# eloimoliner/BABE

Measured on AMD Instinct MI355X. Metric: audio-sec/s (blind BWE, 10 s @ 44.1 kHz clips, 35 EDM steps 2nd order), whole job, higher is better.
Workload: dtype f32

## Files before the change

### babe_amd/_lib.py

```python
import ctypes as C
import os

import torch

_HERE = os.path.dirname(os.path.abspath(__file__))
_LIB_PATH = os.environ.get("BABE_HIP_LIB") or os.path.join(_HERE, "libbabe_hip.so")
_lib = None


class BabeHipError(RuntimeError):
    pass


class ConvArgs(C.Structure):
    _fields_ = [
        ("in_", C.c_void_p), ("in_bs", C.c_long), ("in_cs", C.c_long),
        ("in2", C.c_void_p), ("in2_bs", C.c_long), ("in2_cs", C.c_long), ("cin_split", C.c_int),
        ("w_packed", C.c_void_p),
        ("out", C.c_void_p), ("out_bs", C.c_long), ("out_cs", C.c_long),
        ("res", C.c_void_p), ("res_bs", C.c_long), ("res_cs", C.c_long),
        ("in_scale", C.c_void_p), ("oscale", C.c_void_p),
        ("alpha", C.c_float), ("rbeta", C.c_float),
        ("B", C.c_int), ("Cin", C.c_int), ("Cout", C.c_int), ("F", C.c_int), ("T", C.c_int),
        ("KH", C.c_int), ("KW", C.c_int), ("dil", C.c_int),
# ... 48 lines not shown
    "babe_scale_gelu": [_P, _P, _P, _I, _I, _L, _P],
    "babe_units_size": [_I, _I, _I],
    "babe_scale_gelu_units": [_P, _P, _P, _I, _I, _I, _I, _P],
    "babe_conv2d_bf16_units_supported": [C.POINTER(ConvArgs)],
    "babe_conv2d_bf16_units": [C.POINTER(ConvArgs), _P, _P],
    "babe_gn_bwd_partial": [_P, _P, _P, _P, _I, _I, _I, _L, _I, _P],
    "babe_gn_bwd_apply": [_P, _P, _P, _P, _P, _P, _P, _F, _I, _I, _I, _L, _I, _F, _P],
    "babe_gn_bwd_apply_merge": [_P, _P, _P, _P, _P, _P, _P, _F, _I, _I, _I, _L, _I, _F, _P, _P, _F, _F],
    "babe_gn_bwd_partial_nogelu": [_P, _P, _P, _P, _I, _I, _I, _L, _I, _P],
    "babe_gn_bwd_apply_nogelu": [_P, _P, _P, _P, _P, _P, _P, _F, _I, _I, _I, _L, _I, _F, _P],
    "babe_attn_buckets": [_P, _I, _I, _I],
    "babe_attn_fwd": [_P, _P, _P, _P, _P, _I, _P, _P, _I, _I, _I, _I, _F, _P],
    "babe_attn_vjp": [_P, _P, _P, _P, _P, _I, _P, _P, _P, _P, _P, _P, _I, _I, _I, _I, _F, _P],
    "babe_resample": [_P, _L, _L, _P, _L, _L, _I, _I, _I, _I, _I, _F, _F, _P],
    "babe_resample_res": [_P, _L, _L, _P, _L, _L, _P, _L, _L, _I, _I, _I, _I, _I, _F, _F, _P],
    "babe_resample_sinc_adjoint": [_P, _L, _P, _L, _I, _L, _L, _P, _P, _I, _I, _I, _P],
    "babe_iir_filter": [_P, _L, _P, _L, _I, _L, _P, _P, _I, _I, _I, _P, _L, _P, _L, _P],
    "babe_decimate": [_P, _L, _P, _L, _I, _L, _L, _I, _I, _P],
    "babe_axpby4d": [_P, _L, _L, _P, _L, _L, _I, _I, _I, _I, _F, _F, _P],
    "babe_axpby2_4d": [_P, _L, _L, _P, _L, _L, _P, _L, _L, _I, _I, _I, _I, _F, _F, _P],
    "babe_linear": [_P, _P, _P, _P, _I, _I, _I, _I, _P],
    "babe_rff": [_P, _P, _P, _I, _I, _P],
    "babe_conv_wgrad_rows": [C.POINTER(WgradArgs), _P, _P, _F, _P, _P, _L, _F, _P, _L, _P],
    "babe_rows_sum": [_P, _L, _I, _L, _P, _F, _P],
    "babe_gn_param_grad": [_P, _P, _P, _P, _P, _P, _L, _F, _P, _L, _P, _L, _I, _I, _I, _L, _P],
    "babe_linear_bwd": [_P, _P, _P, _P, _P, _P, _P, _P, _I, _I, _I, _F, _P],
}


def lib():
    global _lib
    if _lib is None:
        if not os.path.exists(_LIB_PATH):
            raise BabeHipError(
# ... 107 lines not shown
```

### babe_amd/csrc/misc.hip

```cpp
#include "common.h"
#include "../../include/babe_hip.h"
#include "prof.h"
#include <cstdarg>
#include <vector>

static thread_local char g_err[512] = "";

void babe_set_error(const char* fmt, ...) {
    va_list ap;
    va_start(ap, fmt);
    vsnprintf(g_err, sizeof(g_err), fmt, ap);
    va_end(ap);
}
extern "C" const char* babe_last_error(void) { return g_err; }
extern "C" const char* babe_version(void) { return "babe_hip 0.1 (gfx950)"; }

namespace {
struct ProfRec { hipEvent_t e0, e1; int slot; void* stream; double flops; };
struct Prof {
    bool on = false;
    int conv_slot_override = -1;
    std::vector<ProfRec> rec;
    size_t used = 0;
    double bytes[BABE_NSLOTS] = {}, flops[BABE_NSLOTS] = {}, exec[BABE_NSLOTS] = {};
// ... 107 lines not shown
                                                      float* __restrict__ out, long out_bs, long out_cs, int C, long n,
                                                      float alpha, float beta) {
    const int b = blockIdx.y / C, c = blockIdx.y % C;
    const float* x = in + (long)b * in_bs + (long)c * in_cs;
    float* y = out + (long)b * out_bs + (long)c * out_cs;
    const long stride = (long)gridDim.x * blockDim.x * V;
    for (long i = ((long)blockIdx.x * blockDim.x + threadIdx.x) * V; i < n; i += stride) {
        if constexpr (V == 4) {
            typedef float f32x4 __attribute__((ext_vector_type(4)));
            f32x4 v = alpha * *reinterpret_cast<const f32x4*>(x + i);
            if (beta != 0.f) v += beta * *reinterpret_cast<const f32x4*>(y + i);
            *reinterpret_cast<f32x4*>(y + i) = v;
        } else {
            const float v = alpha * x[i];
            y[i] = (beta != 0.f) ? v + beta * y[i] : v;
        }
    }
}

__global__ __launch_bounds__(256) void axpby2_4d_kernel(const float* __restrict__ xin, long x_bs, long x_cs,
                                                        const float* __restrict__ yin, long y_bs, long y_cs,
                                                        float* __restrict__ out, long out_bs, long out_cs, int C, long n,
                                                        float alpha, float beta) {
    typedef float f32x4 __attribute__((ext_vector_type(4)));
    const int b = blockIdx.y / C, c = blockIdx.y % C;
    const float* x = xin + (long)b * x_bs + (long)c * x_cs;
    const float* y = yin + (long)b * y_bs + (long)c * y_cs;
    float* o = out + (long)b * out_bs + (long)c * out_cs;
    const long stride = (long)gridDim.x * blockDim.x * 4;
    for (long i = ((long)blockIdx.x * blockDim.x + threadIdx.x) * 4; i < n; i += stride) {
// ... 56 lines not shown
    if (v4) {
        int bx = cdiv(n / 4, 256);
        if (bx > 64) bx = 64;
        hipLaunchKernelGGL(axpby4d_kernel<4>, dim3(bx, B * C), dim3(256), 0, (hipStream_t)stream, in, in_bs, in_cs, out,
                           out_bs, out_cs, C, n, alpha, beta);
    } else {
        int bx = cdiv(n, 256);
        if (bx > 64) bx = 64;
        hipLaunchKernelGGL(axpby4d_kernel<1>, dim3(bx, B * C), dim3(256), 0, (hipStream_t)stream, in, in_bs, in_cs, out,
                           out_bs, out_cs, C, n, alpha, beta);
    }
    BABE_LAUNCH_CHECK();
    return BABE_OK;
}

extern "C" int babe_axpby2_4d(const float* x, long x_bs, long x_cs, const float* y, long y_bs, long y_cs, float* out, long out_bs,
                              long out_cs, int B, int C, int F, int T, float alpha, float beta, void* stream) {
    BABE_CHECK_ARG(x && y && out && B > 0 && C > 0 && F > 0 && T > 0, "axpby2_4d: bad arguments");
    BABE_CHECK_ARG((long)B * C <= 65535, "axpby2_4d: grid too large");
    const long n = (long)F * T;
    auto al16 = [](const void* p) { return ((uintptr_t)p & 15) == 0; };
    BABE_CHECK_ARG(n % 4 == 0 && al16(x) && al16(y) && al16(out) && x_bs % 4 == 0 && x_cs % 4 == 0 && y_bs % 4 == 0 && y_cs % 4 == 0 &&
                       out_bs % 4 == 0 && out_cs % 4 == 0,
                   "axpby2_4d: planes must be 16-byte aligned with F*T %% 4 == 0 (use two babe_axpby4d calls otherwise)");
    BabeProfScope prof(BABE_SLOT_AXPBY, 12.0 * B * C * (double)n, 0, 0, stream);
    int bx = cdiv(n / 4, 256);
    if (bx > 64) bx = 64;
    hipLaunchKernelGGL(axpby2_4d_kernel, dim3(bx, B * C), dim3(256), 0, (hipStream_t)stream, x, x_bs, x_cs, y, y_bs, y_cs, out, out_bs,
                       out_cs, C, n, alpha, beta);
    BABE_LAUNCH_CHECK();
// ... 31 lines not shown
```

### babe_amd/csrc/resample.hip

```cpp
#include "common.h"
#include "../../include/babe_hip.h"
#include "prof.h"

namespace {
__constant__ float kH[8] = {-0.01171875f, -0.03515625f, 0.11328125f, 0.43359375f,
                            0.43359375f,  0.11328125f,  -0.03515625f, -0.01171875f};

__device__ __forceinline__ int refl(int j, int T) { return j < 0 ? -j : (j >= T ? 2 * (T - 1) - j : j); }

__device__ __forceinline__ float down_gpad(const float* gy, int i, int Th) {
    float s = 0.f;
#pragma unroll
    for (int k = 0; k < 8; ++k) {
        const int d = i - k;
        if (d >= 0 && !(d & 1) && (d >> 1) < Th) s += kH[k] * gy[d >> 1];
    }
    return s;
}
__device__ __forceinline__ float up_gpad(const float* gy, int j, int T2) {
    float s = 0.f;
#pragma unroll
    for (int k = 0; k < 8; ++k) {
        const int n = 2 * j + k - 7;
        if (n >= 0 && n < T2) s += kH[k] * gy[n];
// ... 21 lines not shown
        if (n >= 1 && n <= 3) s += down_gpad(x, 3 - n, Th);
        if (n >= T - 4 && n <= T - 2) s += down_gpad(x, 2 * T + 1 - n, Th);
    } else {
        const int T2 = 2 * T;
        s = up_gpad(x, n + 2, T2);
        if (n >= 1 && n <= 2) s += up_gpad(x, 2 - n, T2);
        if (n >= T - 3 && n <= T - 2) s += up_gpad(x, 2 * T - n, T2);
    }
    return s;
}

template <int V, int VI>
__global__ __launch_bounds__(256) void resample_kernel(const float* __restrict__ in, long in_bs, long in_cs,
                                                       float* __restrict__ out, long out_bs, long out_cs, int C, int F,
                                                       int T, int mode, float alpha, float beta, int tout_shift,
                                                       const float* res, long res_bs, long res_cs) {
    const int b = blockIdx.y / C, c = blockIdx.y % C;
    const int Tin = (mode == 0 || mode == 1) ? T : (mode == 2 ? T / 2 : 2 * T);
    const int Tout = (mode == 0) ? T / 2 : (mode == 1 ? 2 * T : T);
    const unsigned i = (blockIdx.x * blockDim.x + threadIdx.x) * (unsigned)V;
    if (i >= (unsigned)(F * Tout)) return;
    const int f = tout_shift >= 0 ? (int)(i >> tout_shift) : (int)(i / (unsigned)Tout);
    const int n0 = (int)(i - (unsigned)f * (unsigned)Tout);
    const float* x = in + (long)b * in_bs + (long)c * in_cs + (long)f * Tin;
    float* y = out + (long)b * out_bs + (long)c * out_cs + (long)f * Tout + n0;
    const float* ry = res ? res + (long)b * res_bs + (long)c * res_cs + (long)f * Tout + n0 : y;
    float s[V];
    if constexpr (V == 4) {
        if (mode == 0 || mode == 3) {
            float w[14];
            const int base = 2 * n0 - 3;
            const bool inner = base >= 0 && base + 13 <= Tin - 1;
            if (inner) {
                if (VI && base - 1 >= 0 && base + 14 <= Tin - 1) {
                    typedef float f32x4 __attribute__((ext_vector_type(4)));
                    const f32x4* p4 = reinterpret_cast<const f32x4*>(x + base - 1);
                    const f32x4 q0 = p4[0], q1 = p4[1], q2 = p4[2], q3 = p4[3];
                    const float X[16] = {q0[0], q0[1], q0[2], q0[3], q1[0], q1[1], q1[2], q1[3],
                                         q2[0], q2[1], q2[2], q2[3], q3[0], q3[1], q3[2], q3[3]};
// ... 102 lines not shown
#pragma unroll
        for (int v = 0; v < V; ++v) s[v] = alpha * resample_one(x, n0 + v, T, mode);
    }
    if constexpr (V == 4) {
        typedef float f32x4 __attribute__((ext_vector_type(4)));
        f32x4 o = {s[0], s[1], s[2], s[3]};
        if (beta != 0.f) o += beta * *reinterpret_cast<const f32x4*>(ry);
        *reinterpret_cast<f32x4*>(y) = o;
    } else {
        y[0] = (beta != 0.f) ? s[0] + beta * ry[0] : s[0];
    }
}
}

static int resample_launch(const float* in, long in_bs, long in_cs, float* out, long out_bs, long out_cs, const float* res,
                           long res_bs, long res_cs, int B, int C, int F, int T, int mode, float alpha, float beta, void* stream) {
    BABE_CHECK_ARG(in && out && B > 0 && C > 0 && F > 0, "resample: bad arguments");
    BABE_CHECK_ARG(!res || ((((uintptr_t)res & 15) == 0) && res_bs % 4 == 0 && res_cs % 4 == 0 && (((uintptr_t)out & 15) == 0) &&
                            out_bs % 4 == 0 && out_cs % 4 == 0),
                   "resample_res: res / out must be 16-byte aligned views");
    BABE_CHECK_ARG(mode >= 0 && mode <= 3, "resample: bad mode %d", mode);
    BABE_CHECK_ARG(T >= 8 && (T % 2) == 0, "resample: T=%d unsupported (need even T >= 8)", T);
    BABE_CHECK_ARG((long)B * C <= 65535, "resample: grid too large");
    const int Tout = (mode == 0) ? T / 2 : (mode == 1 ? 2 * T : T);
    const bool v4 = (Tout % 4 == 0) && (((uintptr_t)out & 15) == 0) && (out_bs % 4 == 0) && (out_cs % 4 == 0);
    const long total = (long)F * Tout;
    BABE_CHECK_ARG(total < (1L << 31), "resample: plane too large");
    int tsh = -1;
    for (int k = 0; k < 31; ++k)
        if ((1 << k) == Tout) tsh = k;
    BabeProfScope prof(BABE_SLOT_RESAMPLE, 4.0 * B * C * (double)F * ((mode == 0 || mode == 1 ? T : (mode == 2 ? T / 2 : 2 * T)) + (beta != 0.f ? 2 : 1) * (double)Tout), 0, 0, stream);
    const int Tin = (mode == 0 || mode == 1) ? T : (mode == 2 ? T / 2 : 2 * T);
    const bool vin = (Tin % 4 == 0) && (((uintptr_t)in & 15) == 0) && (in_bs % 4 == 0) && (in_cs % 4 == 0);
    if (v4 && vin)
        hipLaunchKernelGGL((resample_kernel<4, 1>), dim3(cdiv(total / 4, 256), B * C), dim3(256), 0, (hipStream_t)stream, in,
                           in_bs, in_cs, out, out_bs, out_cs, C, F, T, mode, alpha, beta, tsh, res, res_bs, res_cs);
    else if (v4)
        hipLaunchKernelGGL((resample_kernel<4, 0>), dim3(cdiv(total / 4, 256), B * C), dim3(256), 0, (hipStream_t)stream, in,
                           in_bs, in_cs, out, out_bs, out_cs, C, F, T, mode, alpha, beta, tsh, res, res_bs, res_cs);
    else
        hipLaunchKernelGGL((resample_kernel<1, 0>), dim3(cdiv(total, 256), B * C), dim3(256), 0, (hipStream_t)stream, in,
                           in_bs, in_cs, out, out_bs, out_cs, C, F, T, mode, alpha, beta, tsh, res, res_bs, res_cs);
    BABE_LAUNCH_CHECK();
    return BABE_OK;
}

extern "C" int babe_resample(const float* in, long in_bs, long in_cs, float* out, long out_bs, long out_cs, int B,
                             int C, int F, int T, int mode, float alpha, float beta, void* stream) {
    return resample_launch(in, in_bs, in_cs, out, out_bs, out_cs, nullptr, 0, 0, B, C, F, T, mode, alpha, beta, stream);
}

extern "C" int babe_resample_res(const float* in, long in_bs, long in_cs, const float* res, long res_bs, long res_cs, float* out,
                                 long out_bs, long out_cs, int B, int C, int F, int T, int mode, float alpha, float beta,
                                 void* stream) {
    BABE_CHECK_ARG(res, "resample_res: null res");
    return resample_launch(in, in_bs, in_cs, out, out_bs, out_cs, res, res_bs, res_cs, B, C, F, T, mode, alpha, beta, stream);
}
```

### babe_amd/csrc/unet_engine.hip

```cpp
#include "common.h"
#include "../../include/babe_hip.h"
#include <cmath>
#include <cstdlib>
#include <cstring>

extern "C" int babe_conv2d_auto(babe_conv_args* a, const babe_packed_conv* pc, int transpose, void* stream) {
    BABE_CHECK_ARG(a && pc, "conv2d_auto: null arguments");
    a->Cin = transpose ? pc->Cout : pc->Cin;
    a->Cout = transpose ? pc->Cin : pc->Cout;
    a->KH = pc->KH;
    a->KW = pc->KW;
    const void* wq = transpose ? pc->bwd : pc->fwd;
    BABE_CHECK_ARG(wq, "conv2d_auto: weights not packed for this direction");
    if (!a->in2) a->cin_split = a->Cin;
    if (pc->splits) {
        a->w_packed = nullptr;
        a->stat_mode = 0;
        return babe_conv2d_bf16(a, wq, pc->splits, stream);
    }
    a->w_packed = (const float*)wq;
    const float* w45 = transpose ? pc->bwd_wino45 : pc->fwd_wino45;
    if (pc->w_raw && a->Cout <= 4 && babe_conv2d_fewco_supported(a)) {
        a->stat_mode = 0;
        return babe_conv2d_fewco(a, pc->w_raw, transpose, stream);
// ... 93 lines not shown
        a.B = B(); a.F = x.F; a.T = x.T; a.dil = dil;
        if (stat_part) { a.stat_mode = 1; a.stat_cg = stat_cg; a.stat_part = stat_part; }
        ck(babe_conv2d_auto(&a, &pc, transpose ? 1 : 0, st));
        return a.stat_mode == 1;
    }
    static int stat_slots(int cg, int F, int T, int dil) {
        babe_conv_args a;
        memset(&a, 0, sizeof a);
        a.stat_cg = cg; a.F = F; a.T = T; a.dil = dil;
        return babe_conv2d_wino85_stat_slots(&a);
    }
    void axpby(const View& x, const View& out, float alpha = 1.f, float beta = 0.f) {
        if (dry() || err) return;
        ck(babe_axpby4d(x.p, x.bs, x.cs, out.p, out.bs, out.cs, B(), x.C, x.F, x.T, alpha, beta, st));
    }
    static bool al16(const View& v) { return ((uintptr_t)v.p & 15) == 0 && v.bs % 4 == 0 && v.cs % 4 == 0; }
    void axpby2(const View& x, const View& y, const View& out, float alpha, float beta) {
        if (dry() || err) return;
        if (((long)x.F * x.T) % 4 == 0 && al16(x) && al16(y) && al16(out))
            ck(babe_axpby2_4d(x.p, x.bs, x.cs, y.p, y.bs, y.cs, out.p, out.bs, out.cs, B(), x.C, x.F, x.T, alpha, beta, st));
        else {
            axpby(x, out, alpha);
            axpby(y, out, beta, 1.f);
        }
    }
    void resample(const View& x, const View& out, int mode, float alpha = 1.f, float beta = 0.f, const View* res = nullptr) {
        if (dry() || err) return;
        const int T = mode == 0 || mode == 1 ? x.T : (mode == 2 ? x.T * 2 : x.T / 2);
        if (res) {
            if (al16(*res) && al16(out)) {
                ck(babe_resample_res(x.p, x.bs, x.cs, res->p, res->bs, res->cs, out.p, out.bs, out.cs, B(), x.C, x.F, T, mode, alpha, beta, st));
                return;
            }
            axpby(*res, out);
        }
        ck(babe_resample(x.p, x.bs, x.cs, out.p, out.bs, out.cs, B(), x.C, x.F, T, mode, alpha, beta, st));
    }
    static int splits(long n) { long s = n / 16384; return (int)(s < 1 ? 1 : (s > 64 ? 64 : s)); }
    const float* film_at(int off) const { return S->film + off; }

    View block_fwd(const babe_unet_block& blk, Saved* saved, const View& x, const View& out, const View* x2) {
        const int N = blk.N, Fq = x.F, T = x.T;
        View z;
        if (blk.proj_in.Cout) {
            z = buf(N, Fq, T);
            conv(x, blk.proj_in, z, 1, false, x2, nullptr, nullptr, nullptr, 1.f, 0.f);
        } else if (x.dense()) {
            z = x;
        } else {
            z = buf(N, Fq, T);
            axpby(x, z);
// ... 58 lines not shown
        a.B = B(); a.F = src.F; a.T = src.T; a.dil = dil;
        if (fuse_gn() && blk.k53 && cg % 4 == 0 && z.dense() && da.dense()) {
            a.stat_mode = 2; a.stat_cg = cg; a.stat_x = z.p; a.stat_scale = sv.scale; a.stat_part = *part;
        }
        ck(babe_conv2d_auto(&a, &blk.H[d], 1, st));
        return a.stat_mode == 2 ? Sf : 0;
    }
    static bool fuse_gn_fwd() {
        static const bool on = [] { const char* e = getenv("BABE_FUSE_GN_FWD"); return !(e && atoi(e) == 0); }();
        return on;
    }
    static bool fuse_gn() {
        static const bool on = [] { const char* e = getenv("BABE_FUSE_GN"); return e && atoi(e) != 0; }();
        return on;
    }
    void gn_bwd(const Saved& sv, const View& da, const View& gy, const View& gx, float rbeta, const View* acc, double* part, int Sf) {
        const View& z = sv.z;
        const long n = (long)(z.C / G_GROUPS) * z.F * z.T;
        const int Sp = Sf > 0 ? Sf : splits(n);
        if (dry() || err) return;
        if (Sf <= 0) ck(babe_gn_bwd_partial(z.p, da.p, sv.scale, part, B(), z.C, G_GROUPS, (long)z.F * z.T, Sp, st));
        if (acc)
            ck(babe_gn_bwd_apply_merge(z.p, da.p, gy.p, sv.scale, sv.stats, part, gx.p, rbeta, B(), z.C, G_GROUPS, (long)z.F * z.T, Sp, GN_EPS, st,
                                       acc->p, RS2, RS2));
        else
            ck(babe_gn_bwd_apply(z.p, da.p, gy.p, sv.scale, sv.stats, part, gx.p, rbeta, B(), z.C, G_GROUPS, (long)z.F * z.T, Sp, GN_EPS, st));
    }
    View block_vjp(const babe_unet_block& blk, const Saved* saved, const View& g_out, const View& g_in, bool accumulate, bool consume) {
        const int N = blk.N, Fq = g_out.F, T = g_out.T;
        const float beta = accumulate ? 1.f : 0.f;
        auto da_view = [&]() { View v; v.p = scratch_a((size_t)B() * N * Fq * T); v.C = N; v.F = Fq; v.T = T; v.cs = (long)Fq * T; v.bs = (long)N * Fq * T; return v; };
        if (!blk.res_conv.Cout && !blk.proj_out.Cout && !blk.proj_in.Cout && !accumulate && blk.nd > 0 && g_out.dense()) {
            View gz;
            if (blk.nd > 1) gz = buf(N, Fq, T);
            View da = da_view();
            View src = g_out;
            const bool merged = g_in.dense() && al16(g_in) && al16(g_out);
            for (int d = blk.nd - 1; d >= 0; --d) {
                double* part;
// ... 12 lines not shown
        if (blk.res_conv.Cout) conv(g_out, blk.res_conv, g_in, 1, true, nullptr, accumulate ? &g_in : nullptr, nullptr, nullptr, RS2, beta);
        else axpby(g_out, g_in, RS2, beta);
        float c = 1.f;
        View gz;
        if (blk.proj_out.Cout) {
            gz = buf(N, Fq, T);
            conv(g_out, blk.proj_out, gz, 1, true, nullptr, nullptr, nullptr, nullptr, RS2, 0.f);
        } else if (consume && g_out.dense()) {
            gz = g_out;
            c = RS2;
        } else {
            gz = buf(N, Fq, T);
            axpby(g_out, gz, RS2);
        }
        View da = da_view();
        for (int d = blk.nd - 1; d >= 0; --d) {
            double* part;
            const int Sf = conv_vjp(gz, blk, d, da, saved[d], &part);
            gn_bwd(saved[d], da, gz, gz, RS2, nullptr, part, Sf);
        }
        if (blk.proj_in.Cout) conv(gz, blk.proj_in, g_in, 1, true, nullptr, &g_in, nullptr, nullptr, c, 1.f);
        else axpby(gz, g_in, c, 1.f);
        return g_in;
    }

    void forward(const float* const* C_in, float** outs) {
        const int n = P->nocts, bpo = P->bpo;
        const int* Ns = P->Ns;
        const int* Ts = S->Ts;
        auto cview = [&](int lvl) { View v; v.p = const_cast<float*>(C_in[n - 1 - lvl]); v.C = 2; v.F = bpo; v.T = Ts[lvl]; v.cs = (long)bpo * Ts[lvl]; v.bs = 2 * v.cs; return v; };
        View XC = buf(Ns[0], bpo, Ts[0]);
        View pyr_prev, X;
        for (int i = 0; i < n; ++i) {
            const View C = cview(i);
            const int Fi = bpo * (i + 1);
            block_fwd(P->init_blk[i], S->saved[0][i], C, sub_f(XC, 0, bpo), nullptr);
            View pyr;
// ... 27 lines not shown
        {
            View Xm = buf(X.C, X.F, X.T);
            block_fwd(P->mid_blk, S->saved[4][0], X, Xm, nullptr);
            X = Xm;
        }
        View Xout = buf(2, bpo * n, Ts[n - 1]);
        block_fwd(P->mid_out, S->saved[5][0], X, Xout, nullptr);
        for (int i = 0; i < n; ++i) {
            const int j = n - 1 - i;
            const int Fj = bpo * (j + 1);
            const int Nout = Ns[j > 0 ? j - 1 : 0];
            View R = buf(Nout, Fj, Ts[j]);
            block_fwd(P->up_blk[i], S->saved[3][i], X, R, &S->hs[j]);
            View O = buf(2, Fj, Ts[j]);
            block_fwd(P->up_out[i], S->saved[2][i], R, O, nullptr);
            axpby(O, Xout, RS2, RS2);
            View o; o.p = outs[i]; o.C = 2; o.F = bpo; o.T = Ts[j]; o.cs = (long)bpo * Ts[j]; o.bs = 2 * o.cs;
            axpby(sub_f(Xout, 0, bpo), o);
            if (j > 0) {
                View Xn = buf(Nout, Fj - bpo, Ts[j - 1]);
                resample(sub_f(R, bpo, Fj - bpo), Xn, 1);
                View Xo = buf(2, Fj - bpo, Ts[j - 1]);
                resample(sub_f(Xout, bpo, Fj - bpo), Xo, 1);
                X = Xn;
                Xout = Xo;
            }
        }
    }

    void vjp(const float* const* gouts, float** gC) {
        const int n = P->nocts, bpo = P->bpo;
        const int* Ns = P->Ns;
        const int* Ts = S->Ts;
        View gH[8];
        View gX_prev, gXO_prev;
        for (int j = 0; j < n; ++j) {
            const int i = n - 1 - j;
            const int Fj = bpo * (j + 1);
            const int Nout = Ns[j > 0 ? j - 1 : 0];
            View gXOn = buf(2, Fj, Ts[j]);
            View gcat = buf(2 * Ns[j], Fj, Ts[j]);
            const size_t lvl = mark();
            View gXOp = buf(2, Fj, Ts[j]);
            View go; go.p = const_cast<float*>(gouts[i]); go.C = 2; go.F = bpo; go.T = Ts[j]; go.cs = (long)bpo * Ts[j]; go.bs = 2 * go.cs;
            axpby(go, sub_f(gXOp, 0, bpo));
            View gR = buf(Nout, Fj, Ts[j]);
            bool accumulate = false;
            if (j > 0) {
                resample(gXO_prev, sub_f(gXOp, bpo, Fj - bpo), 3);
                if (!dry() && !err) ck(babe_fill4d(gR.p, gR.bs, gR.cs, B(), Nout, bpo, Ts[j], 0.f, st));
                resample(gX_prev, sub_f(gR, bpo, Fj - bpo), 3);
                accumulate = true;
            }
            View gO = buf(2, Fj, Ts[j]);
            axpby(gXOp, gO, RS2);
            block_vjp(P->up_out[i], S->saved[2][i], gO, gR, accumulate, true);
            axpby(gXOp, gXOn, RS2);
            gXO_prev = gXOn;
            block_vjp(P->up_blk[i], S->saved[3][i], gR, gcat, false, true);
            gX_prev = sub_c(gcat, 0, Ns[j]);
            gH[j] = sub_c(gcat, Ns[j], Ns[j]);
            release(lvl);
        }
        View gM = buf(Ns[n - 1], bpo * n, Ts[n - 1]);
        axpby(gX_prev, gM);
        block_vjp(P->mid_out, S->saved[5][0], gXO_prev, gM, true, true);
        View gXm = buf(gM.C, gM.F, gM.T);
        block_vjp(P->mid_blk, S->saved[4][0], gM, gXm, false, true);
        View gpyr_next, gP;
        bool have_next = false;
        for (int i = n - 1; i >= 0; --i) {
            const int Fi = bpo * (i + 1);
// ... 128 lines not shown
```

### babe_amd/networks/unet_engine.py

```python
import math
import os

import torch

from .. import ops

RS2 = 1.0 / math.sqrt(2.0)
USE_C = os.environ.get("BABE_UNET_C", "0") == "1"
MERGE_TAIL = os.environ.get("BABE_MERGE_TAIL", "1") != "0"


class _Attn:

    def __init__(self, g, Fdim, N, film_index, opts):
        self.H, self.bias_qkv, self.rel_pos, self.nbk, self.maxd = opts
        self.F = Fdim
        self.scale = float(Fdim) ** -0.5
        self.gamma = g("norm2.gamma").reshape(-1).contiguous()
        self.film_off = (film_index.add(g("affine2.weight"), g("affine2.bias")), film_index.add(g("gate2.weight"), g("gate2.bias")))
        self.proj_in = ops.PackedConv(g("attn_block.proj_in.weight"))
        self.proj_out = ops.PackedConv(g("attn_block.proj_out.weight"))
        w = g("attn_block.qk.weight")
        self.qk = ops.PackedConv(w.reshape(w.shape[0], w.shape[1], 1, 1))
        self.qk_bias = g("attn_block.qk.bias").contiguous() if self.bias_qkv else None
# ... 356 lines not shown
            blk.saved = None
            blk.inp = blk.zpo = None
            return g_in
        if blk.res_conv is not None:
            ops.conv2d(g_out, blk.res_conv, g_in, transpose=True, alpha=RS2, rbeta=beta, res=g_in if accumulate else None)
        else:
            ops.axpby(g_out, g_in, alpha=RS2, beta=beta)
        c = 1.0
        if blk.proj_out is not None:
            gz = ops.conv2d(g_out, blk.proj_out, self.buf(B, N, Fq, T), transpose=True, alpha=RS2)
        elif consume and g_out.is_contiguous():
            gz, c = g_out, RS2
        else:
            gz = ops.axpby(g_out, self.buf(B, N, Fq, T), alpha=RS2)
        da = self.scratch("a", B * N * Fq * T).view(B, N, Fq, T)
        for d in reversed(range(blk.nd)):
            z, stats, scale, gate = blk.saved[d]
            if pg is not None:
                self._layer_wgrad(pg, blk, d, gz, c)
            fs = ops.conv2d(gz, blk.H[d], da, dil=blk.dil(d), transpose=True, in_scale=gate, alpha=RS2, vjp_stat=(z, scale, N // 8))
            if pg is not None:
                self._layer_gn_grad(pg, blk, d, da, c)
            ops.gn_bwd(z, da, gz, scale, stats, gz, RS2, fused=fs)
        if blk.attn is not None:
            self.attn_vjp(blk, gz, c)
            c = 1.0
        if pg is not None and blk.proj_in is not None:
            x, x2 = blk.inp
            self._wg(pg, blk.p + "proj_in.weight", x, gz, blk.proj_in, c, x2=x2)
        if blk.proj_in is not None:
            ops.conv2d(gz, blk.proj_in, g_in, transpose=True, res=g_in, alpha=c, rbeta=1.0)
        else:
            ops.axpby(gz, g_in, alpha=c, beta=1.0)
        blk.saved = None
        blk.inp = blk.zpo = None
        return g_in

    def _c_engine(self):
        if not USE_C or self.precision != "f32" or self.has_attention:
            return None
        cu = self.__dict__.get("_cunet")
        if cu is None:
            from .unet_c import CUnet
            parent = self.__dict__.get("_cunet_parent")
            cu = parent.clone(self) if parent is not None else CUnet(self)
            self._cunet = cu
        return cu
# ... 39 lines not shown
                ops.resample(H, sub, 0)
                ops.conv2d(pyr, self.pyr_conv[i], sub, res=sub, alpha=RS2, rbeta=RS2)
                XC = XCn
            else:
                X = ops.conv2d(pyr, self.pyr_conv[i], self.buf(B, Ns[i], Fi, Ts[i]), res=H, alpha=RS2, rbeta=RS2)
        self.hs = hs
        X = self.block_fwd(self.mid_blk, X, film, self.buf(*X.shape))
        Xout = self.block_fwd(self.mid_out, X, film, self.buf(B, 2, bpo * n, Ts[-1]))
        outs = [None] * n
        for i in range(n):
            j = n - 1 - i
            Fj = bpo * (j + 1)
            Nout = Ns[max(j - 1, 0)]
            R = self.block_fwd(self.up_blk[i], X, film, self.buf(B, Nout, Fj, Ts[j]), x2=hs[j])
            O = self.block_fwd(self.up_out[i], R, film, self.buf(B, 2, Fj, Ts[j]))
            ops.axpby(O, Xout, alpha=RS2, beta=RS2)
            outs[i] = ops.axpby(Xout[:, :, :bpo, :], self.buf(B, 2, bpo, Ts[j]))
            if j > 0:
                X = ops.resample(R[:, :, bpo:, :], self.buf(B, Nout, Fj - bpo, Ts[j - 1]), 1)
                Xout = ops.resample(Xout[:, :, bpo:, :], self.buf(B, 2, Fj - bpo, Ts[j - 1]), 1)
        return outs

    def vjp(self, gouts, pg=None):
        assert pg is None or self._train, "parameter gradients need forward(..., train=True)"
        if getattr(self, "_c_fwd", False):
            return self._c_engine().vjp([g.contiguous() for g in gouts])
        n, bpo, Ns, Ts, B = self.nocts, self.bpo, self.Ns, self.Ts, self.B
        gH = [None] * n
        gX_prev = gXO_prev = None
        for j in range(n):
            i = n - 1 - j
            Fj = bpo * (j + 1)
            Nout = Ns[max(j - 1, 0)]
            gXOp = self.buf(B, 2, Fj, Ts[j])
            ops.axpby(gouts[i], gXOp[:, :, :bpo, :])
            gR = self.buf(B, Nout, Fj, Ts[j])
            if j > 0:
                ops.resample(gXO_prev, gXOp[:, :, bpo:, :], 3)
                gR[:, :, :bpo, :].zero_()
                ops.resample(gX_prev, gR[:, :, bpo:, :], 3)
                accumulate = True
            else:
                accumulate = False
            gO = ops.axpby(gXOp, self.buf(B, 2, Fj, Ts[j]), alpha=RS2)
            self.block_vjp(self.up_out[i], gO, gR, accumulate=accumulate, consume=True, pg=pg)
            gXO_prev = ops.axpby(gXOp, self.buf(B, 2, Fj, Ts[j]), alpha=RS2)
            gcat = self.buf(B, 2 * Ns[j], Fj, Ts[j])
            self.block_vjp(self.up_blk[i], gR, gcat, consume=True, pg=pg)
            gX_prev = gcat[:, :Ns[j]]
            gH[j] = gcat[:, Ns[j]:]
        gM = self.buf(B, Ns[-1], bpo * n, Ts[-1])
        ops.axpby(gX_prev, gM)
        self.block_vjp(self.mid_out, gXO_prev, gM, accumulate=True, consume=True, pg=pg)
        gXm = self.block_vjp(self.mid_blk, gM, self.buf(*gM.shape), consume=True, pg=pg)
        gC = [None] * n
        gpyr_next = None
        gP = None
        for i in reversed(range(n)):
            Fi = bpo * (i + 1)
            if pg is not None:
                self._wg(pg, f"downs.{i}.1.weight", self.pyrs[i], gXm if i == n - 1 else gP, self.pyr_conv[i], RS2)
# ... 28 lines not shown
```

### babe_amd/ops.py

```python
import ctypes as C
import math
import os

import torch

from . import _lib
from ._lib import ConvArgs, CPackedConv, WgradArgs, check, lib, ptr, stream

RSQRT2 = 1.0 / math.sqrt(2.0)


def _view(t):
    assert t.dim() == 4 and t.dtype == torch.float32
    assert t.stride(3) == 1 and t.stride(2) == t.shape[3], f"rows must be contiguous, got strides {t.stride()}"
    return ptr(t), t.stride(0), t.stride(1)


PRECISIONS = {"f32": 0, "bf16": 1, "bf16x3": 2}
BF16_HBM_F32 = os.environ.get("BABE_BF16_HBM_F32", "1") != "0"
_W = os.environ.get("BABE_CONV_WINO", "4")
FEWCO = os.environ.get("BABE_CONV_FEWCO", "1") != "0"
WINOGRAD = _W != "0"
WINOGRAD4 = _W not in ("0", "2", "1")
WINOGRAD45 = WINOGRAD4 and os.environ.get("BABE_CONV_WINO45", "1") != "0"
# ... 326 lines not shown
    assert out.shape == (B, Cc, F, Tout), (out.shape, (B, Cc, F, Tout))
    xp, xbs, xcs = _view(x)
    op, obs, ocs = _view(out)
    if res is not None:
        assert res.shape == out.shape
        rp, rbs, rcs = _view(res)
        if AXPBY2 and all(v % 4 == 0 for v in (rbs, rcs, obs, ocs)) and res.data_ptr() % 16 == 0 and out.data_ptr() % 16 == 0:
            check(lib().babe_resample_res(xp, xbs, xcs, rp, rbs, rcs, op, obs, ocs, B, Cc, F, T, mode, alpha, beta, stream()),
                  "resample_res")
            return out
        axpby(res, out)
    check(lib().babe_resample(xp, xbs, xcs, op, obs, ocs, B, Cc, F, T, mode, alpha, beta, stream()), "resample")
    return out


def axpby(x, out, alpha=1.0, beta=0.0):
    assert x.shape == out.shape
    B, Cc, F, T = x.shape
    xp, xbs, xcs = _view(x)
    op, obs, ocs = _view(out)
    check(lib().babe_axpby4d(xp, xbs, xcs, op, obs, ocs, B, Cc, F, T, alpha, beta, stream()), "axpby4d")
    return out


def axpby2(x, y, out, alpha, beta):
    assert x.shape == out.shape and y.shape == out.shape
    B, Cc, F, T = x.shape
    xp, xbs, xcs = _view(x)
    yp, ybs, ycs = _view(y)
    op, obs, ocs = _view(out)
# ... 146 lines not shown
```

### include/babe_hip.h

```cpp
#ifndef BABE_HIP_H
#define BABE_HIP_H
#ifdef __cplusplus
extern "C" {
#endif

const char* babe_version(void);
const char* babe_last_error(void);

typedef struct { float* p; long bs; long cs; } babe_view;

typedef struct {
    const float* in;  long in_bs,  in_cs;
    const float* in2; long in2_bs, in2_cs; int cin_split;
    const float* w_packed;
    float* out;       long out_bs, out_cs;
    const float* res; long res_bs, res_cs;
    const float* in_scale;
    const float* oscale;
    float alpha, rbeta;
    int B, Cin, Cout, F, T, KH, KW, dil;
    int stat_mode, stat_cg;
    const float* stat_x; const float* stat_scale; double* stat_part;
} babe_conv_args;
int babe_conv2d_wino85_stat_slots(const babe_conv_args* a);
// ... 55 lines not shown
                      int B, int C, int G, long hw, int S, float eps, void* stream);
int babe_gn_bwd_apply_merge(const float* x, const float* da, const float* gy, const float* scale,
                            const float* stats, const double* part, float* gx, float rbeta,
                            int B, int C, int G, long hw, int S, float eps, void* stream,
                            const float* acc, float ca, float cb);
int babe_gn_bwd_partial_nogelu(const float* x, const float* da, const float* scale, double* part, int B, int C, int G, long hw,
                               int S, void* stream);
int babe_gn_bwd_apply_nogelu(const float* x, const float* da, const float* gy, const float* scale, const float* stats,
                             const double* part, float* gx, float rbeta, int B, int C, int G, long hw, int S, float eps,
                             void* stream);

int babe_resample(const float* in, long in_bs, long in_cs, float* out, long out_bs, long out_cs,
                  int B, int C, int F, int T, int mode, float alpha, float beta, void* stream);
int babe_resample_res(const float* in, long in_bs, long in_cs, const float* res, long res_bs, long res_cs, float* out,
                      long out_bs, long out_cs, int B, int C, int F, int T, int mode, float alpha, float beta, void* stream);

int babe_resample_sinc(const float* x, long x_bs, float* out, long out_bs, int B, long L_in, long L_out, const float* kernel,
                       const int* krange, int orig, int new_, int width, void* stream);
int babe_resample_sinc_adjoint(const float* g, long g_bs, float* out, long out_bs, int B, long L_in, long L_out,
                               const float* kernel, const int* krange, int orig, int new_, int width, void* stream);

long babe_iir_workspace(int B, long L, int order);
int babe_iir_filter(const float* x, long x_bs, float* y, long y_bs, int B, long L, const float* b, const float* a, int order,
                    int clamp, int adjoint, unsigned char* mask, long mask_bs, void* workspace, long workspace_bytes, void* stream);
int babe_decimate(const float* in, long in_bs, float* out, long out_bs, int B, long L_full, long L_dec, int factor, int adjoint,
                  void* stream);

long babe_conv_packed_size_wino85(int Cout, int Cin, int transpose_flip);
int babe_conv_pack_weights_wino85(const float* w, float* dst, int Cout, int Cin, int KH, int KW, int transpose_flip, void* stream);
int babe_conv2d_wino85_supported(const babe_conv_args* a);
// ... 20 lines not shown
    int Ns[8];
    babe_unet_block init_blk[8], main_blk[8], up_out[8], up_blk[8], mid_blk, mid_out;
    babe_packed_conv pyr_conv[8];
} babe_unet_plan_desc;
void* babe_unet_plan_create(const babe_unet_plan_desc* desc);
void babe_unet_plan_destroy(void* plan);
void* babe_unet_state_create(void);
void babe_unet_state_destroy(void* state);
long babe_unet_workspace_bytes(const void* plan, int B, const int* T_oct);
int babe_unet_fwd(const void* plan, void* state, const float* const* C_in, const float* film, long film_bs, int B,
                  const int* T_oct, void* workspace, long workspace_bytes, float* const* outs, void* stream);
int babe_unet_vjp(const void* plan, void* state, const float* const* gouts, float* const* gC, void* stream);

int babe_axpby4d(const float* in, long in_bs, long in_cs, float* out, long out_bs, long out_cs,
                 int B, int C, int F, int T, float alpha, float beta, void* stream);
int babe_fill4d(float* out, long out_bs, long out_cs, int B, int C, int F, int T, float value, void* stream);
int babe_axpby2_4d(const float* x, long x_bs, long x_cs, const float* y, long y_bs, long y_cs, float* out, long out_bs,
                   long out_cs, int B, int C, int F, int T, float alpha, float beta, void* stream);

int babe_linear(const float* x, const float* W, const float* bias, float* out, int B, int K, int J,
                int relu, void* stream);
int babe_rff(const float* cnoise, const float* freq, float* out, int B, int R, void* stream);

int babe_rfft_mixed(const float* x_in, float* spec_out, const float* spec_in, float* x_out, float* work, int B, int N1,
                    int N2, int K2, const int* rad1, int nrad1, const int* rad2, int nrad2, const float* w1, const float* w2,
                    const float* tw, int direction, void* stream);
int babe_fft_twiddle_transpose(const float* in, float* out, const float* tw, int B, int N1, int N2,
                               int adjoint, void* stream);
typedef struct {
    int nbands; int L; int KX;
// ... 156 lines not shown
```

Baseline: 2.548.

## Fuse elementwise copies, zero-fill and tail axpby into neighbouring UNet kernels

Several small elementwise passes in the UNet forward and VJP are folded into adjacent kernels. The output-add and copy-out become a single dual-store axpby. The zero-fill of the leading rows joins the upsampling resample. The RS2 scale moves into the gradient copy and resample, which removes two temporary buffers. The final residual axpby in the block VJP is merged into the last group-norm backward apply. These changes cut kernel launches and memory traffic, at the cost of more special-case code paths and argument plumbing that must stay correct.

```diff
diff --git a/babe_amd/_lib.py b/babe_amd/_lib.py
--- a/babe_amd/_lib.py
+++ b/babe_amd/_lib.py
@@ -86,10 +86,12 @@
     "babe_attn_vjp": [_P, _P, _P, _P, _P, _I, _P, _P, _P, _P, _P, _P, _I, _I, _I, _I, _F, _P],
     "babe_resample": [_P, _L, _L, _P, _L, _L, _I, _I, _I, _I, _I, _F, _F, _P],
     "babe_resample_res": [_P, _L, _L, _P, _L, _L, _P, _L, _L, _I, _I, _I, _I, _I, _F, _F, _P],
+    "babe_resample_zrows": [_P, _L, _L, _P, _L, _L, _I, _I, _I, _I, _I, _F, _I, _P],
     "babe_resample_sinc_adjoint": [_P, _L, _P, _L, _I, _L, _L, _P, _P, _I, _I, _I, _P],
     "babe_iir_filter": [_P, _L, _P, _L, _I, _L, _P, _P, _I, _I, _I, _P, _L, _P, _L, _P],
     "babe_decimate": [_P, _L, _P, _L, _I, _L, _L, _I, _I, _P],
     "babe_axpby4d": [_P, _L, _L, _P, _L, _L, _I, _I, _I, _I, _F, _F, _P],
+    "babe_axpby4d_dup": [_P, _L, _L, _P, _L, _L, _P, _L, _L, _I, _I, _I, _I, _I, _F, _F, _P],
     "babe_axpby2_4d": [_P, _L, _L, _P, _L, _L, _P, _L, _L, _I, _I, _I, _I, _F, _F, _P],
     "babe_linear": [_P, _P, _P, _P, _I, _I, _I, _I, _P],
     "babe_rff": [_P, _P, _P, _I, _I, _P],
diff --git a/babe_amd/csrc/misc.hip b/babe_amd/csrc/misc.hip
--- a/babe_amd/csrc/misc.hip
+++ b/babe_amd/csrc/misc.hip
@@ -145,6 +145,32 @@
         } else {
             const float v = alpha * x[i];
             y[i] = (beta != 0.f) ? v + beta * y[i] : v;
+        }
+    }
+}
+
+template <int V>
+__global__ __launch_bounds__(256) void axpby4d_dup_kernel(const float* __restrict__ in, long in_bs, long in_cs,
+                                                          float* __restrict__ out, long out_bs, long out_cs,
+                                                          float* __restrict__ out2, long out2_bs, long out2_cs, int C, long n,
+                                                          long n2, float alpha, float beta) {
+    const int b = blockIdx.y / C, c = blockIdx.y % C;
+    const float* x = in + (long)b * in_bs + (long)c * in_cs;
+    float* y = out + (long)b * out_bs + (long)c * out_cs;
+    float* y2 = out2 + (long)b * out2_bs + (long)c * out2_cs;
+    const long stride = (long)gridDim.x * blockDim.x * V;
+    for (long i = ((long)blockIdx.x * blockDim.x + threadIdx.x) * V; i < n; i += stride) {
+        if constexpr (V == 4) {
+            typedef float f32x4 __attribute__((ext_vector_type(4)));
+            f32x4 v = alpha * *reinterpret_cast<const f32x4*>(x + i);
+            if (beta != 0.f) v += beta * *reinterpret_cast<const f32x4*>(y + i);
+            *reinterpret_cast<f32x4*>(y + i) = v;
+            if (i < n2) *reinterpret_cast<f32x4*>(y2 + i) = v;
+        } else {
+            float v = alpha * x[i];
+            if (beta != 0.f) v = v + beta * y[i];
+            y[i] = v;
+            if (i < n2) y2[i] = v;
         }
     }
 }
@@ -231,6 +257,30 @@
     return BABE_OK;
 }
 
+extern "C" int babe_axpby4d_dup(const float* in, long in_bs, long in_cs, float* out, long out_bs, long out_cs, float* out2,
+                                long out2_bs, long out2_cs, int B, int C, int F, int T, int F2, float alpha, float beta, void* stream) {
+    BABE_CHECK_ARG(in && out && out2 && B > 0 && C > 0 && F > 0 && T > 0 && F2 > 0 && F2 <= F, "axpby4d_dup: bad arguments");
+    BABE_CHECK_ARG((long)B * C <= 65535 && F <= 65535, "axpby4d_dup: grid too large");
+    const long n = (long)F * T, n2 = (long)F2 * T;
+    auto al16 = [](const void* p) { return ((uintptr_t)p & 15) == 0; };
+    const bool v4 = (n % 4 == 0) && (n2 % 4 == 0) && al16(in) && al16(out) && al16(out2) && in_bs % 4 == 0 && in_cs % 4 == 0 &&
+                    out_bs % 4 == 0 && out_cs % 4 == 0 && out2_bs % 4 == 0 && out2_cs % 4 == 0;
+    BabeProfScope prof(BABE_SLOT_AXPBY, ((beta != 0.f ? 12.0 : 8.0) * (double)n + 4.0 * (double)n2) * B * C, 0, 0, stream);
+    if (v4) {
+        int bx = cdiv(n / 4, 256);
+        if (bx > 64) bx = 64;
+        hipLaunchKernelGGL(axpby4d_dup_kernel<4>, dim3(bx, B * C), dim3(256), 0, (hipStream_t)stream, in, in_bs, in_cs, out,
+                           out_bs, out_cs, out2, out2_bs, out2_cs, C, n, n2, alpha, beta);
+    } else {
+        int bx = cdiv(n, 256);
+        if (bx > 64) bx = 64;
+        hipLaunchKernelGGL(axpby4d_dup_kernel<1>, dim3(bx, B * C), dim3(256), 0, (hipStream_t)stream, in, in_bs, in_cs, out,
+                           out_bs, out_cs, out2, out2_bs, out2_cs, C, n, n2, alpha, beta);
+    }
+    BABE_LAUNCH_CHECK();
+    return BABE_OK;
+}
+
 extern "C" int babe_axpby2_4d(const float* x, long x_bs, long x_cs, const float* y, long y_bs, long y_cs, float* out, long out_bs,
                               long out_cs, int B, int C, int F, int T, float alpha, float beta, void* stream) {
     BABE_CHECK_ARG(x && y && out && B > 0 && C > 0 && F > 0 && T > 0, "axpby2_4d: bad arguments");
diff --git a/babe_amd/csrc/resample.hip b/babe_amd/csrc/resample.hip
--- a/babe_amd/csrc/resample.hip
+++ b/babe_amd/csrc/resample.hip
@@ -59,15 +59,25 @@
 __global__ __launch_bounds__(256) void resample_kernel(const float* __restrict__ in, long in_bs, long in_cs,
                                                        float* __restrict__ out, long out_bs, long out_cs, int C, int F,
                                                        int T, int mode, float alpha, float beta, int tout_shift,
-                                                       const float* res, long res_bs, long res_cs) {
+                                                       const float* res, long res_bs, long res_cs, int zrows) {
     const int b = blockIdx.y / C, c = blockIdx.y % C;
     const int Tin = (mode == 0 || mode == 1) ? T : (mode == 2 ? T / 2 : 2 * T);
     const int Tout = (mode == 0) ? T / 2 : (mode == 1 ? 2 * T : T);
     const unsigned i = (blockIdx.x * blockDim.x + threadIdx.x) * (unsigned)V;
-    if (i >= (unsigned)(F * Tout)) return;
+    if (i >= (unsigned)((F + zrows) * Tout)) return;
     const int f = tout_shift >= 0 ? (int)(i >> tout_shift) : (int)(i / (unsigned)Tout);
     const int n0 = (int)(i - (unsigned)f * (unsigned)Tout);
-    const float* x = in + (long)b * in_bs + (long)c * in_cs + (long)f * Tin;
+    if (f < zrows) {
+        float* z = out + (long)b * out_bs + (long)c * out_cs + (long)f * Tout + n0;
+        if constexpr (V == 4) {
+            typedef float f32x4 __attribute__((ext_vector_type(4)));
+            *reinterpret_cast<f32x4*>(z) = f32x4{0.f, 0.f, 0.f, 0.f};
+        } else {
+            z[0] = 0.f;
+        }
+        return;
+    }
+    const float* x = in + (long)b * in_bs + (long)c * in_cs + (long)(f - zrows) * Tin;
     float* y = out + (long)b * out_bs + (long)c * out_cs + (long)f * Tout + n0;
     const float* ry = res ? res + (long)b * res_bs + (long)c * res_cs + (long)f * Tout + n0 : y;
     float s[V];
@@ -200,7 +210,8 @@
 }
 
 static int resample_launch(const float* in, long in_bs, long in_cs, float* out, long out_bs, long out_cs, const float* res,
-                           long res_bs, long res_cs, int B, int C, int F, int T, int mode, float alpha, float beta, void* stream) {
+                           long res_bs, long res_cs, int B, int C, int F, int T, int mode, float alpha, float beta, void* stream,
+                           int zrows = 0) {
     BABE_CHECK_ARG(in && out && B > 0 && C > 0 && F > 0, "resample: bad arguments");
     BABE_CHECK_ARG(!res || ((((uintptr_t)res & 15) == 0) && res_bs % 4 == 0 && res_cs % 4 == 0 && (((uintptr_t)out & 15) == 0) &&
                             out_bs % 4 == 0 && out_cs % 4 == 0),
@@ -210,7 +221,7 @@
     BABE_CHECK_ARG((long)B * C <= 65535, "resample: grid too large");
     const int Tout = (mode == 0) ? T / 2 : (mode == 1 ? 2 * T : T);
     const bool v4 = (Tout % 4 == 0) && (((uintptr_t)out & 15) == 0) && (out_bs % 4 == 0) && (out_cs % 4 == 0);
-    const long total = (long)F * Tout;
+    const long total = (long)(F + zrows) * Tout;
     BABE_CHECK_ARG(total < (1L << 31), "resample: plane too large");
     int tsh = -1;
     for (int k = 0; k < 31; ++k)
@@ -220,13 +231,13 @@
     const bool vin = (Tin % 4 == 0) && (((uintptr_t)in & 15) == 0) && (in_bs % 4 == 0) && (in_cs % 4 == 0);
     if (v4 && vin)
         hipLaunchKernelGGL((resample_kernel<4, 1>), dim3(cdiv(total / 4, 256), B * C), dim3(256), 0, (hipStream_t)stream, in,
-                           in_bs, in_cs, out, out_bs, out_cs, C, F, T, mode, alpha, beta, tsh, res, res_bs, res_cs);
+                           in_bs, in_cs, out, out_bs, out_cs, C, F, T, mode, alpha, beta, tsh, res, res_bs, res_cs, zrows);
     else if (v4)
         hipLaunchKernelGGL((resample_kernel<4, 0>), dim3(cdiv(total / 4, 256), B * C), dim3(256), 0, (hipStream_t)stream, in,
-                           in_bs, in_cs, out, out_bs, out_cs, C, F, T, mode, alpha, beta, tsh, res, res_bs, res_cs);
+                           in_bs, in_cs, out, out_bs, out_cs, C, F, T, mode, alpha, beta, tsh, res, res_bs, res_cs, zrows);
     else
         hipLaunchKernelGGL((resample_kernel<1, 0>), dim3(cdiv(total, 256), B * C), dim3(256), 0, (hipStream_t)stream, in,
-                           in_bs, in_cs, out, out_bs, out_cs, C, F, T, mode, alpha, beta, tsh, res, res_bs, res_cs);
+                           in_bs, in_cs, out, out_bs, out_cs, C, F, T, mode, alpha, beta, tsh, res, res_bs, res_cs, zrows);
     BABE_LAUNCH_CHECK();
     return BABE_OK;
 }
@@ -242,3 +253,9 @@
     BABE_CHECK_ARG(res, "resample_res: null res");
     return resample_launch(in, in_bs, in_cs, out, out_bs, out_cs, res, res_bs, res_cs, B, C, F, T, mode, alpha, beta, stream);
 }
+
+extern "C" int babe_resample_zrows(const float* in, long in_bs, long in_cs, float* out, long out_bs, long out_cs, int B, int C, int F,
+                                   int T, int mode, float alpha, int zrows, void* stream) {
+    BABE_CHECK_ARG(zrows >= 0, "resample_zrows: bad zrows");
+    return resample_launch(in, in_bs, in_cs, out, out_bs, out_cs, nullptr, 0, 0, B, C, F, T, mode, alpha, 0.f, stream, zrows);
+}
diff --git a/babe_amd/csrc/unet_engine.hip b/babe_amd/csrc/unet_engine.hip
--- a/babe_amd/csrc/unet_engine.hip
+++ b/babe_amd/csrc/unet_engine.hip
@@ -131,6 +131,10 @@
         if (dry() || err) return;
         ck(babe_axpby4d(x.p, x.bs, x.cs, out.p, out.bs, out.cs, B(), x.C, x.F, x.T, alpha, beta, st));
     }
+    void axpby_dup(const View& x, const View& out, const View& out2, float alpha, float beta) {
+        if (dry() || err) return;
+        ck(babe_axpby4d_dup(x.p, x.bs, x.cs, out.p, out.bs, out.cs, out2.p, out2.bs, out2.cs, B(), x.C, x.F, x.T, out2.F, alpha, beta, st));
+    }
     static bool al16(const View& v) { return ((uintptr_t)v.p & 15) == 0 && v.bs % 4 == 0 && v.cs % 4 == 0; }
     void axpby2(const View& x, const View& y, const View& out, float alpha, float beta) {
         if (dry() || err) return;
@@ -152,6 +156,11 @@
             axpby(*res, out);
         }
         ck(babe_resample(x.p, x.bs, x.cs, out.p, out.bs, out.cs, B(), x.C, x.F, T, mode, alpha, beta, st));
+    }
+    void resample_zrows(const View& x, const View& out, int mode, int zrows, float alpha = 1.f) {
+        if (dry() || err) return;
+        const int T = mode == 0 || mode == 1 ? x.T : (mode == 2 ? x.T * 2 : x.T / 2);
+        ck(babe_resample_zrows(x.p, x.bs, x.cs, out.p, out.bs, out.cs, B(), x.C, x.F, T, mode, alpha, zrows, st));
     }
     static int splits(long n) { long s = n / 16384; return (int)(s < 1 ? 1 : (s > 64 ? 64 : s)); }
     const float* film_at(int off) const { return S->film + off; }
@@ -240,7 +249,8 @@
         static const bool on = [] { const char* e = getenv("BABE_FUSE_GN"); return e && atoi(e) != 0; }();
         return on;
     }
-    void gn_bwd(const Saved& sv, const View& da, const View& gy, const View& gx, float rbeta, const View* acc, double* part, int Sf) {
+    void gn_bwd(const Saved& sv, const View& da, const View& gy, const View& gx, float rbeta, const View* acc, double* part, int Sf,
+                float ca = RS2, float cb = RS2) {
         const View& z = sv.z;
         const long n = (long)(z.C / G_GROUPS) * z.F * z.T;
         const int Sp = Sf > 0 ? Sf : splits(n);
@@ -248,7 +258,7 @@
         if (Sf <= 0) ck(babe_gn_bwd_partial(z.p, da.p, sv.scale, part, B(), z.C, G_GROUPS, (long)z.F * z.T, Sp, st));
         if (acc)
             ck(babe_gn_bwd_apply_merge(z.p, da.p, gy.p, sv.scale, sv.stats, part, gx.p, rbeta, B(), z.C, G_GROUPS, (long)z.F * z.T, Sp, GN_EPS, st,
-                                       acc->p, RS2, RS2));
+                                       acc->p, ca, cb));
         else
             ck(babe_gn_bwd_apply(z.p, da.p, gy.p, sv.scale, sv.stats, part, gx.p, rbeta, B(), z.C, G_GROUPS, (long)z.F * z.T, Sp, GN_EPS, st));
     }
@@ -291,13 +301,15 @@
             axpby(g_out, gz, RS2);
         }
         View da = da_view();
+        const bool tail_merged = !blk.proj_in.Cout && blk.nd > 0 && g_in.C == N && g_in.dense() && al16(g_in);
         for (int d = blk.nd - 1; d >= 0; --d) {
             double* part;
             const int Sf = conv_vjp(gz, blk, d, da, saved[d], &part);
-            gn_bwd(saved[d], da, gz, gz, RS2, nullptr, part, Sf);
+            if (d == 0 && tail_merged) gn_bwd(saved[d], da, gz, g_in, RS2, &g_in, part, Sf, 1.f, c);
+            else gn_bwd(saved[d], da, gz, gz, RS2, nullptr, part, Sf);
         }
         if (blk.proj_in.Cout) conv(gz, blk.proj_in, g_in, 1, true, nullptr, &g_in, nullptr, nullptr, c, 1.f);
-        else axpby(gz, g_in, c, 1.f);
+        else if (!tail_merged) axpby(gz, g_in, c, 1.f);
         return g_in;
     }
 
@@ -355,9 +367,8 @@
             block_fwd(P->up_blk[i], S->saved[3][i], X, R, &S->hs[j]);
             View O = buf(2, Fj, Ts[j]);
             block_fwd(P->up_out[i], S->saved[2][i], R, O, nullptr);
-            axpby(O, Xout, RS2, RS2);
             View o; o.p = outs[i]; o.C = 2; o.F = bpo; o.T = Ts[j]; o.cs = (long)bpo * Ts[j]; o.bs = 2 * o.cs;
-            axpby(sub_f(Xout, 0, bpo), o);
+            axpby_dup(O, Xout, o, RS2, RS2);
             if (j > 0) {
                 View Xn = buf(Nout, Fj - bpo, Ts[j - 1]);
                 resample(sub_f(R, bpo, Fj - bpo), Xn, 1);
@@ -382,21 +393,16 @@
             View gXOn = buf(2, Fj, Ts[j]);
             View gcat = buf(2 * Ns[j], Fj, Ts[j]);
             const size_t lvl = mark();
-            View gXOp = buf(2, Fj, Ts[j]);
             View go; go.p = const_cast<float*>(gouts[i]); go.C = 2; go.F = bpo; go.T = Ts[j]; go.cs = (long)bpo * Ts[j]; go.bs = 2 * go.cs;
-            axpby(go, sub_f(gXOp, 0, bpo));
+            axpby(go, sub_f(gXOn, 0, bpo), RS2);
             View gR = buf(Nout, Fj, Ts[j]);
             bool accumulate = false;
             if (j > 0) {
-                resample(gXO_prev, sub_f(gXOp, bpo, Fj - bpo), 3);
-                if (!dry() && !err) ck(babe_fill4d(gR.p, gR.bs, gR.cs, B(), Nout, bpo, Ts[j], 0.f, st));
-                resample(gX_prev, sub_f(gR, bpo, Fj - bpo), 3);
+                resample(gXO_prev, sub_f(gXOn, bpo, Fj - bpo), 3, RS2);
+                resample_zrows(gX_prev, gR, 3, bpo);
                 accumulate = true;
             }
-            View gO = buf(2, Fj, Ts[j]);
-            axpby(gXOp, gO, RS2);
-            block_vjp(P->up_out[i], S->saved[2][i], gO, gR, accumulate, true);
-            axpby(gXOp, gXOn, RS2);
+            block_vjp(P->up_out[i], S->saved[2][i], gXOn, gR, accumulate, false);
             gXO_prev = gXOn;
             block_vjp(P->up_blk[i], S->saved[3][i], gR, gcat, false, true);
             gX_prev = sub_c(gcat, 0, Ns[j]);
diff --git a/babe_amd/networks/unet_engine.py b/babe_amd/networks/unet_engine.py
--- a/babe_amd/networks/unet_engine.py
+++ b/babe_amd/networks/unet_engine.py
@@ -394,6 +394,8 @@
         else:
             gz = ops.axpby(g_out, self.buf(B, N, Fq, T), alpha=RS2)
         da = self.scratch("a", B * N * Fq * T).view(B, N, Fq, T)
+        tail_merged = (blk.proj_in is None and blk.attn is None and blk.nd > 0 and g_in.shape[1] == N and g_in.is_contiguous()
+                       and g_in.data_ptr() % 16 == 0)
         for d in reversed(range(blk.nd)):
             z, stats, scale, gate = blk.saved[d]
             if pg is not None:
@@ -401,7 +403,10 @@
             fs = ops.conv2d(gz, blk.H[d], da, dil=blk.dil(d), transpose=True, in_scale=gate, alpha=RS2, vjp_stat=(z, scale, N // 8))
             if pg is not None:
                 self._layer_gn_grad(pg, blk, d, da, c)
-            ops.gn_bwd(z, da, gz, scale, stats, gz, RS2, fused=fs)
+            if d == 0 and tail_merged:
+                ops.gn_bwd(z, da, gz, scale, stats, g_in, RS2, merge=(g_in, 1.0, c), fused=fs)
+            else:
+                ops.gn_bwd(z, da, gz, scale, stats, gz, RS2, fused=fs)
         if blk.attn is not None:
             self.attn_vjp(blk, gz, c)
             c = 1.0
@@ -410,7 +415,7 @@
             self._wg(pg, blk.p + "proj_in.weight", x, gz, blk.proj_in, c, x2=x2)
         if blk.proj_in is not None:
             ops.conv2d(gz, blk.proj_in, g_in, transpose=True, res=g_in, alpha=c, rbeta=1.0)
-        else:
+        elif not tail_merged:
             ops.axpby(gz, g_in, alpha=c, beta=1.0)
         blk.saved = None
         blk.inp = blk.zpo = None
@@ -480,8 +485,8 @@
             Nout = Ns[max(j - 1, 0)]
             R = self.block_fwd(self.up_blk[i], X, film, self.buf(B, Nout, Fj, Ts[j]), x2=hs[j])
             O = self.block_fwd(self.up_out[i], R, film, self.buf(B, 2, Fj, Ts[j]))
-            ops.axpby(O, Xout, alpha=RS2, beta=RS2)
-            outs[i] = ops.axpby(Xout[:, :, :bpo, :], self.buf(B, 2, bpo, Ts[j]))
+            outs[i] = self.buf(B, 2, bpo, Ts[j])
+            ops.axpby_dup(O, Xout, outs[i], alpha=RS2, beta=RS2)
             if j > 0:
                 X = ops.resample(R[:, :, bpo:, :], self.buf(B, Nout, Fj - bpo, Ts[j - 1]), 1)
                 Xout = ops.resample(Xout[:, :, bpo:, :], self.buf(B, 2, Fj - bpo, Ts[j - 1]), 1)
@@ -498,19 +503,17 @@
             i = n - 1 - j
             Fj = bpo * (j + 1)
             Nout = Ns[max(j - 1, 0)]
-            gXOp = self.buf(B, 2, Fj, Ts[j])
-            ops.axpby(gouts[i], gXOp[:, :, :bpo, :])
+            gXOn = self.buf(B, 2, Fj, Ts[j])
+            ops.axpby(gouts[i], gXOn[:, :, :bpo, :], alpha=RS2)
             gR = self.buf(B, Nout, Fj, Ts[j])
             if j > 0:
-                ops.resample(gXO_prev, gXOp[:, :, bpo:, :], 3)
-                gR[:, :, :bpo, :].zero_()
-                ops.resample(gX_prev, gR[:, :, bpo:, :], 3)
+                ops.resample(gXO_prev, gXOn[:, :, bpo:, :], 3, alpha=RS2)
+                ops.resample_zrows(gX_prev, gR, 3, bpo)
                 accumulate = True
             else:
                 accumulate = False
-            gO = ops.axpby(gXOp, self.buf(B, 2, Fj, Ts[j]), alpha=RS2)
-            self.block_vjp(self.up_out[i], gO, gR, accumulate=accumulate, consume=True, pg=pg)
-            gXO_prev = ops.axpby(gXOp, self.buf(B, 2, Fj, Ts[j]), alpha=RS2)
+            self.block_vjp(self.up_out[i], gXOn, gR, accumulate=accumulate, pg=pg)
+            gXO_prev = gXOn
             gcat = self.buf(B, 2 * Ns[j], Fj, Ts[j])
             self.block_vjp(self.up_blk[i], gR, gcat, consume=True, pg=pg)
             gX_prev = gcat[:, :Ns[j]]
diff --git a/babe_amd/ops.py b/babe_amd/ops.py
--- a/babe_amd/ops.py
+++ b/babe_amd/ops.py
@@ -364,6 +364,28 @@
     return out
 
 
+def resample_zrows(x, out, mode, zrows, alpha=1.0):
+    B, Cc, F, Tin = x.shape
+    T = {0: Tin, 1: Tin, 2: Tin * 2, 3: Tin // 2}[mode]
+    Tout = {0: T // 2, 1: 2 * T, 2: T, 3: T}[mode]
+    assert out.shape == (B, Cc, F + zrows, Tout), (out.shape, (B, Cc, F + zrows, Tout))
+    xp, xbs, xcs = _view(x)
+    op, obs, ocs = _view(out)
+    check(lib().babe_resample_zrows(xp, xbs, xcs, op, obs, ocs, B, Cc, F, T, mode, alpha, zrows, stream()), "resample_zrows")
+    return out
+
+
+def axpby_dup(x, out, out2, alpha=1.0, beta=0.0):
+    assert x.shape == out.shape and out2.shape[:2] == out.shape[:2] and out2.shape[3] == out.shape[3] and out2.shape[2] <= out.shape[2]
+    B, Cc, F, T = x.shape
+    xp, xbs, xcs = _view(x)
+    op, obs, ocs = _view(out)
+    o2p, o2bs, o2cs = _view(out2)
+    check(lib().babe_axpby4d_dup(xp, xbs, xcs, op, obs, ocs, o2p, o2bs, o2cs, B, Cc, F, T, out2.shape[2], alpha, beta, stream()),
+          "axpby4d_dup")
+    return out
+
+
 def axpby(x, out, alpha=1.0, beta=0.0):
     assert x.shape == out.shape
     B, Cc, F, T = x.shape
diff --git a/include/babe_hip.h b/include/babe_hip.h
--- a/include/babe_hip.h
+++ b/include/babe_hip.h
@@ -93,6 +93,8 @@
                   int B, int C, int F, int T, int mode, float alpha, float beta, void* stream);
 int babe_resample_res(const float* in, long in_bs, long in_cs, const float* res, long res_bs, long res_cs, float* out,
                       long out_bs, long out_cs, int B, int C, int F, int T, int mode, float alpha, float beta, void* stream);
+int babe_resample_zrows(const float* in, long in_bs, long in_cs, float* out, long out_bs, long out_cs, int B, int C, int F,
+                        int T, int mode, float alpha, int zrows, void* stream);
 
 int babe_resample_sinc(const float* x, long x_bs, float* out, long out_bs, int B, long L_in, long L_out, const float* kernel,
                        const int* krange, int orig, int new_, int width, void* stream);
@@ -143,6 +145,8 @@
 
 int babe_axpby4d(const float* in, long in_bs, long in_cs, float* out, long out_bs, long out_cs,
                  int B, int C, int F, int T, float alpha, float beta, void* stream);
+int babe_axpby4d_dup(const float* in, long in_bs, long in_cs, float* out, long out_bs, long out_cs, float* out2, long out2_bs,
+                     long out2_cs, int B, int C, int F, int T, int F2, float alpha, float beta, void* stream);
 int babe_fill4d(float* out, long out_bs, long out_cs, int B, int C, int F, int T, float value, void* stream);
 int babe_axpby2_4d(const float* x, long x_bs, long x_cs, const float* y, long y_bs, long y_cs, float* out, long out_bs,
                    long out_cs, int B, int C, int F, int T, float alpha, float beta, void* stream);
```

Result: no change. 2.558 (median of 6 runs) (+0.4%).
